# jedison-github/gentun

Measured on AMD Instinct MI355X. Metric: candidates/hour + best val-acc@genN, Genetic-CNN CIFAR-10 1/2/4/8 GPU, higher is better.
Workload: dtype fp32

## Files before the change

### csrc/hip/cnn_dense.hip

```cpp

#include <algorithm>
#include <cstdlib>

#include "common.h"

#define HEAD_MAXC_FWD 16
#define ADAM_B1 0.9f
#define ADAM_B2 0.999f
#define ADAM_EPS 1e-7f
#define CLIP_EPS 1e-7f
#define GT_DGRAD_BUF 2
#define GT_ADAM_UNROLL 1

__global__ void step_begin_kernel(StepState* s) {
  s->cur_step = s->step_ctr;
  s->step_ctr += 1;
  s->global_step += 1;
  const float t = s->t + 1.0f;
  s->t = t;
  s->lr_t = s->opt == 1 ? s->lr : s->lr * sqrtf(1.0f - powf(ADAM_B2, t)) / (1.0f - powf(ADAM_B1, t));
}

struct DenseFwdArgs {
  const void* x;
// ... 245 lines not shown
  const StepState* st;
  float* dH;
  float* gw2;
  float* gb2;
  float* gb1;
  float* eval_out;
  float* dz;
  const float* plog;
  int G, B, Up, C;
  int loss_ce;
  float drop_scale;
  int eval;
  int prec;
  const int* valid;
  const int* valid_norm;
  uint16_t* dHp;
};

#define HEAD_MAXB 64
#define HEAD_MAXC 16

__global__ void __launch_bounds__(64) head_fwd_kernel(HeadArgs a) {
  const int idx = blockIdx.x, lane = threadIdx.x;
  const int g = idx / a.B, b = idx % a.B;
  const int C = a.C, nt = a.Up / 16;
  const int step = a.st ? a.st->cur_step : 0;
  const long sid = a.gather[((long)step * a.G + g) * a.B + b];
  const int y = (int)a.labels[sid];
  float acc[HEAD_MAXC];
  const float* pl = a.plog + ((long)g * nt * a.B + b) * C;
#pragma unroll
  for (int c = 0; c < HEAD_MAXC; ++c) acc[c] = 0.f;
  for (int t = lane; t < nt; t += 64) {
    float v[HEAD_MAXC];
#pragma unroll
    for (int c = 0; c < HEAD_MAXC; ++c) v[c] = pl[(long)t * a.B * C + min(c, C - 1)];
#pragma unroll
    for (int c = 0; c < HEAD_MAXC; ++c) acc[c] += c < C ? v[c] : 0.f;
  }
#pragma unroll
  for (int c = 0; c < HEAD_MAXC; ++c) {
    if (c < C) {
#pragma unroll
      for (int o = 32; o > 0; o >>= 1) acc[c] += __shfl_xor(acc[c], o);
    }
  }
  if (lane != 0) return;
  float logit[HEAD_MAXC];
  for (int c = 0; c < C; ++c) logit[c] = acc[c] + a.b2[(long)g * C + c];
  float p[HEAD_MAXC];
  float mx = -INFINITY;
  for (int c = 0; c < C; ++c) mx = fmaxf(mx, logit[c]);
  float z = 0.f;
  for (int c = 0; c < C; ++c) { p[c] = expf(logit[c] - mx); z += p[c]; }
  int arg = 0;
  float loss = 0.f, binc = 0.f;
  for (int c = 0; c < C; ++c) {
    p[c] /= z;
    if (p[c] > p[arg]) arg = c;
    const float yc = (c == y) ? 1.f : 0.f;
    binc += (rintf(p[c]) == yc) ? 1.f : 0.f;
    if (!a.loss_ce) {
      const float pc = fminf(fmaxf(p[c], CLIP_EPS), 1.f - CLIP_EPS);
      loss += -(yc * logf(pc) + (1.f - yc) * logf(1.f - pc)) / C;
    }
  }
  if (a.loss_ce) loss = -logf(fmaxf(p[y], 1e-30f));
  if (a.eval) {
    float* e = a.eval_out + ((long)g * a.B + b) * 3;
    e[0] = loss; e[1] = binc; e[2] = (arg == y) ? 1.f : 0.f;
    return;
  }
  float* dz = a.dz + ((long)g * a.B + b) * C;
  const int nv = a.valid ? a.valid[(long)step * a.G + g] : a.B;
  const int nn = a.valid_norm ? a.valid_norm[(long)step * a.G + g] : nv;
  const float inv_b = (b < nv && nn > 0) ? 1.0f / nn : 0.f;
  if (a.loss_ce) {
    for (int c = 0; c < C; ++c) dz[c] = (p[c] - ((c == y) ? 1.f : 0.f)) * inv_b;
  } else {
    float dp[HEAD_MAXC], s = 0.f;
    for (int c = 0; c < C; ++c) {
      const float yc = (c == y) ? 1.f : 0.f;
      const bool inside = p[c] >= CLIP_EPS && p[c] <= 1.f - CLIP_EPS;
      const float pc = fminf(fmaxf(p[c], CLIP_EPS), 1.f - CLIP_EPS);
      dp[c] = inside ? (pc - yc) / (pc * (1.f - pc)) / C : 0.f;
      s += p[c] * dp[c];
    }
    for (int c = 0; c < C; ++c) dz[c] = p[c] * (dp[c] - s) * inv_b;
  }
}

__global__ void __launch_bounds__(256) head_bwd_kernel(HeadArgs a) {
  __shared__ float dzs[HEAD_MAXB * HEAD_MAXC];
  __shared__ float w2s[64 * HEAD_MAXC];
  __shared__ float hsl[HEAD_MAXB][65];
  __shared__ float colsum[4][64];
  const int g = blockIdx.y, u0 = blockIdx.x * 64, tid = threadIdx.x;
  const int B = a.B, Up = a.Up, C = a.C;
  const float* dz = a.dz + (long)g * B * C;
  for (int i = tid; i < B * C; i += 256) dzs[i] = dz[i];
  for (int i = tid; i < 64 * C; i += 256) {
    const int u = u0 + i / C;
    w2s[i] = (u < Up) ? a.w2[((long)g * Up + u0) * C + i] : 0.f;
  }
  for (int i = tid; i < B * 64; i += 256) {
    const int b = i >> 6, j = i & 63;
    const long hi = ((long)g * B + b) * Up + u0 + j;
    hsl[b][j] = (u0 + j < Up) ? (a.prec ? static_cast<const float*>(a.h)[hi] : bf2f(static_cast<const uint16_t*>(a.h)[hi]))
                              : 0.f;
  }
  __syncthreads();
  {
    const int j = tid & 63, q = tid >> 6;
    float sb = 0.f;
    for (int b = q; b < B; b += 4) {
      float s = 0.f;
      for (int c = 0; c < C; ++c) s += dzs[b * C + c] * w2s[j * C + c];
      const float d = hsl[b][j] > 0.f ? s * a.drop_scale : 0.f;
      if (u0 + j < Up) {
        const long o = ((long)g * B + b) * Up + u0 + j;
        a.dH[o] = d;
        if (a.dHp) {
          if (a.prec) {
            uint16_t hq[3];
            split3(d, hq);
            const long ps = (long)a.G * B * Up;
            a.dHp[o] = hq[0]; a.dHp[ps + o] = hq[1]; a.dHp[2 * ps + o] = hq[2];
          } else {
            a.dHp[o] = f2bf(d);
          }
        }
      }
      sb += d;
    }
    colsum[q][j] = sb;
  }
  for (int o = tid; o < 64 * C; o += 256) {
    const int j = o / C, c = o % C;
    if (u0 + j >= Up) continue;
    float s = 0.f;
    for (int b = 0; b < B; ++b) s += hsl[b][j] * dzs[b * C + c];
    a.gw2[((long)g * Up + u0) * C + o] = s;
  }
  __syncthreads();
  if (tid < 64 && u0 + tid < Up)
    a.gb1[(long)g * Up + u0 + tid] = colsum[0][tid] + colsum[1][tid] + colsum[2][tid] + colsum[3][tid];
  if (blockIdx.x == 0 && tid < C) {
    float s = 0.f;
    for (int b = 0; b < B; ++b) s += dzs[b * C + tid];
    a.gb2[(long)g * C + tid] = s;
  }
}

struct DenseDgradArgs {
  const float* dH;
  const void* wt;
  void* dx;
  int G, B, Fp, Up;
  int prec;
  long wps;
  const uint8_t* unpool_mask;
  void* unpool_x0;
  void* unpool_x1;
  const int* unpool_sel;
  int Hs, Ws, Cp;
  const float* w1;
  const uint16_t* dHp;
};

template <int PREC>
__device__ __forceinline__ void dense_dgrad_epilogue(const DenseDgradArgs& a, int g, int f_t, int b0,
                                                     const f32x4_t (&acc)[2], int lane) {
  typedef typename ActT<PREC>::T AT;
  const int kq = lane >> 4, l16 = lane & 15;
  const int fo = f_t + kq * 4;
  if (fo >= a.Fp) return;
#pragma unroll
  for (int h = 0; h < 2; ++h) {
    const int row = b0 + h * 16 + l16;
    if (row >= a.B) continue;
    float v[4] = {acc[h][0], acc[h][1], acc[h][2], acc[h][3]};
    if (a.unpool_mask) {
      const long n = (long)g * a.B + row;
      const int pix = fo / a.Cp, c0 = fo - pix * a.Cp, wo_n = a.Ws >> 1;
      const int ho = pix / wo_n, wo = pix - ho * wo_n;
      const uint32_t mk = *reinterpret_cast<const uint32_t*>(a.unpool_mask + n * a.Fp + fo);
      AT* src = static_cast<AT*>((a.unpool_sel && a.unpool_sel[g]) ? a.unpool_x1 : a.unpool_x0);
#pragma unroll
      for (int me = 0; me < 4; ++me) {
        float o[4];
#pragma unroll
        for (int j = 0; j < 4; ++j) {
          const uint32_t bb = (mk >> (8 * j)) & 0xffu;
          o[j] = ((int)(bb & 3u) == me && (bb & 4u)) ? v[j] : 0.f;
        }
        AT* d = src + ((n * a.Hs + 2 * ho + (me >> 1)) * a.Ws + 2 * wo + (me & 1)) * a.Cp + c0;
        if (PREC) *reinterpret_cast<float4*>(d) = make_float4(o[0], o[1], o[2], o[3]);
        else *reinterpret_cast<uint2*>(d) = pack4(o);
      }
      continue;
    }
    AT* dst = static_cast<AT*>(a.dx) + ((long)g * a.B + row) * a.Fp + fo;
    if (PREC) *reinterpret_cast<float4*>(dst) = make_float4(v[0], v[1], v[2], v[3]);
    else *reinterpret_cast<uint2*>(dst) = pack4(v);
  }
}

template <int PREC>
__global__ void __launch_bounds__(256) dense_dgrad_stream2_kernel(DenseDgradArgs a) {
  constexpr int NPL = PREC ? GT_NPL_F32 : 1;
  const int tid = threadIdx.x, wave = tid >> 6, lane = tid & 63, kq = lane >> 4, l16 = lane & 15;
  int bx, g;
  xcd_tile(bx, g);
  const int f_t = bx * 128 + wave * 32;
  const int b0 = blockIdx.y * 32;
  const float* wrow[2];
  bool fok[2];
#pragma unroll
  for (int m = 0; m < 2; ++m) {
    const int fa = f_t + 16 * m + l16;
    fok[m] = fa < a.Fp;
    wrow[m] = a.w1 + ((long)g * a.Fp + (fok[m] ? fa : 0)) * a.Up;
  }
  const long ps = (long)a.G * a.B * a.Up;
  const int br[2] = {b0 + l16, b0 + 16 + l16};
  const uint16_t* hp[2];
  bool bok[2];
#pragma unroll
  for (int h = 0; h < 2; ++h) {
    bok[h] = br[h] < a.B;
    hp[h] = a.dHp + ((long)g * a.B + (bok[h] ? br[h] : 0)) * a.Up;
  }
  const int nchunks = a.Up >> 3;
  const int nks = (nchunks + 3) >> 2;
  f32x4_t acc[2][2];
#pragma unroll
  for (int m = 0; m < 2; ++m) acc[m][0] = acc[m][1] = (f32x4_t){0.f, 0.f, 0.f, 0.f};
  constexpr int NBUF = GT_DGRAD_BUF;
  float rw[NBUF][2][8];
  uint4 rh[NBUF][2][NPL];
  const uint4* zero4 = reinterpret_cast<const uint4*>(gt_zero8);
  auto load = [&](int j, int buf) {
    const int c = 4 * j + kq;
    const bool cok = c < nchunks;
#pragma unroll
    for (int m = 0; m < 2; ++m) ld8_raw(wrow[m] + c * 8, cok && fok[m], rw[buf][m]);
#pragma unroll
    for (int h = 0; h < 2; ++h)
#pragma unroll
      for (int p = 0; p < NPL; ++p)
        rh[buf][h][p] = *((cok && bok[h]) ? reinterpret_cast<const uint4*>(hp[h] + p * ps + c * 8) : zero4);
  };
  auto step = [&](int buf) {
#pragma unroll
    for (int m = 0; m < 2; ++m) {
      uint4 af[NPL];
      planes8<PREC>(rw[buf][m], af);
      acc[m][0] = mfma_np<NPL>(af, rh[buf][0], acc[m][0]);
      acc[m][1] = mfma_np<NPL>(af, rh[buf][1], acc[m][1]);
    }
  };
#pragma unroll
  for (int t = 0; t < NBUF; ++t) {
    load(t, t);
    __builtin_amdgcn_sched_barrier(0);
  }
  const int nks2 = (nks + 1) & ~1;
  for (int j = 0; j < nks; j += NBUF) {
#pragma unroll
    for (int t = 0; t < NBUF; ++t) {
      if (j + t < nks2) step(t);
      __builtin_amdgcn_sched_barrier(0);
      load(j + NBUF + t, t);
      __builtin_amdgcn_sched_barrier(0);
    }
  }
#pragma unroll
  for (int m = 0; m < 2; ++m) dense_dgrad_epilogue<PREC>(a, g, f_t + 16 * m, b0, acc[m], lane);
}


__device__ __forceinline__ f32x4_t mfma4f(float a, float b, f32x4_t c) {
  return __builtin_amdgcn_mfma_f32_16x16x4f32(a, b, c, 0, 0, 0);
}

__global__ void __launch_bounds__(256) dense_dgrad_f32_kernel(DenseDgradArgs a) {
  const int tid = threadIdx.x, wave = tid >> 6, lane = tid & 63, kq = lane >> 4, l16 = lane & 15;
  int bx, g;
  xcd_tile(bx, g);
  const int f_t = bx * 128 + wave * 32;
  const int b0 = blockIdx.y * 32;
  const float* wrow[2];
#pragma unroll
  for (int m = 0; m < 2; ++m) wrow[m] = a.w1 + ((long)g * a.Fp + min(f_t + 16 * m + l16, a.Fp - 1)) * a.Up + 8 * kq;
  const float* hrow[2];
#pragma unroll
  for (int h = 0; h < 2; ++h) hrow[h] = a.dH + ((long)g * a.B + min(b0 + 16 * h + l16, a.B - 1)) * a.Up + 8 * kq;
  f32x4_t acc[2][2];
#pragma unroll
  for (int m = 0; m < 2; ++m) acc[m][0] = acc[m][1] = (f32x4_t){0.f, 0.f, 0.f, 0.f};
  constexpr int NB = 2;
  float4 wv[NB][2][2], hv[NB][2][2];
  const int nblk = a.Up >> 5;
  auto load = [&](int j, int buf) {
    const int jj = min(j, nblk - 1);
#pragma unroll
    for (int m = 0; m < 2; ++m) {
      wv[buf][m][0] = *reinterpret_cast<const float4*>(wrow[m] + 32 * jj);
      wv[buf][m][1] = *reinterpret_cast<const float4*>(wrow[m] + 32 * jj + 4);
    }
#pragma unroll
    for (int h = 0; h < 2; ++h) {
      hv[buf][h][0] = *reinterpret_cast<const float4*>(hrow[h] + 32 * jj);
      hv[buf][h][1] = *reinterpret_cast<const float4*>(hrow[h] + 32 * jj + 4);
    }
  };
  auto step = [&](int buf) {
#pragma unroll
    for (int q = 0; q < 8; ++q) {
      const float w0 = (&wv[buf][0][q >> 2].x)[q & 3], w1 = (&wv[buf][1][q >> 2].x)[q & 3];
      const float h0 = (&hv[buf][0][q >> 2].x)[q & 3], h1 = (&hv[buf][1][q >> 2].x)[q & 3];
      acc[0][0] = mfma4f(w0, h0, acc[0][0]);
      acc[0][1] = mfma4f(w0, h1, acc[0][1]);
      acc[1][0] = mfma4f(w1, h0, acc[1][0]);
      acc[1][1] = mfma4f(w1, h1, acc[1][1]);
    }
  };
#pragma unroll
  for (int i = 0; i < NB - 1; ++i) load(i, i);
  for (int j = 0; j < nblk; j += NB) {
#pragma unroll
    for (int q = 0; q < NB; ++q) {
      if (j + q >= nblk) break;
      load(j + q + NB - 1, (q + NB - 1) % NB);
      step(q);
    }
  }
#pragma unroll
  for (int m = 0; m < 2; ++m) dense_dgrad_epilogue<1>(a, g, f_t + 16 * m, b0, acc[m], lane);
}

struct DenseWgradAdamArgs {
  const void* x;
  const float* dH;
  float* p; float* m; float* v;
  void* wt;
  const StepState* st;
  int G, B, Fp, Up;
  int Cp, Cr, Ur;
  int prec;
  long wps;
  float* gbuf;
  int mode;
};

template <int PREC>
__global__ void __launch_bounds__(256) dense_wgrad_adam_kernel(DenseWgradAdamArgs a) {
  typedef typename ActT<PREC>::T AT;
  extern __shared__ __attribute__((aligned(16))) char smem[];
  float* xs = reinterpret_cast<float*>(smem);
  const int g = blockIdx.y, f0 = blockIdx.x * 16, tid = threadIdx.x;
  const AT* x = static_cast<const AT*>(a.x) + (long)g * a.B * a.Fp;
  for (int i = tid; i < a.B * 16; i += 256) {
    const int b = i >> 4, j = i & 15;
    float xv = 0.f;
    if (f0 + j < a.Fp) {
      if (PREC) xv = static_cast<const float*>(static_cast<const void*>(x))[(long)b * a.Fp + f0 + j];
      else xv = bf2f(static_cast<const uint16_t*>(static_cast<const void*>(x))[(long)b * a.Fp + f0 + j]);
    }
    xs[i] = xv;
  }
  __syncthreads();
  const float lr_t = a.st->lr_t;
  const float* dH = a.dH + (long)g * a.B * a.Up;
  const int nq = a.Ur > 0 ? (a.Ur + 3) >> 2 : a.Up >> 2;
  const int fr = tid >> 7;
  for (int q = tid & 127; q < nq; q += 128) {
    const int u0 = q * 4;
    float acc[8][4];
#pragma unroll
    for (int r = 0; r < 8; ++r) acc[r][0] = acc[r][1] = acc[r][2] = acc[r][3] = 0.f;
    if (a.mode == 2) {
#pragma unroll
      for (int r = 0; r < 8; ++r) {
        const int f = f0 + fr + 2 * r;
        if (f < a.Fp) {
          const float4 q4 = *reinterpret_cast<const float4*>(a.gbuf + ((long)g * a.Fp + f) * a.Up + u0);
          acc[r][0] = q4.x; acc[r][1] = q4.y; acc[r][2] = q4.z; acc[r][3] = q4.w;
        }
      }
    }
    for (int b = 0; a.mode != 2 && b < a.B; ++b) {
      const float4 d = *reinterpret_cast<const float4*>(dH + (long)b * a.Up + u0);
#pragma unroll
      for (int r = 0; r < 8; ++r) {
        const float xv = xs[b * 16 + fr + 2 * r];
        acc[r][0] += xv * d.x; acc[r][1] += xv * d.y; acc[r][2] += xv * d.z; acc[r][3] += xv * d.w;
      }
    }
    if (a.mode == 1) {
#pragma unroll
      for (int r = 0; r < 8; ++r) {
        const int f = f0 + fr + 2 * r;
        if (f < a.Fp)
          *reinterpret_cast<float4*>(a.gbuf + ((long)g * a.Fp + f) * a.Up + u0) =
              make_float4(acc[r][0], acc[r][1], acc[r][2], acc[r][3]);
      }
      continue;
    }
#pragma unroll
    for (int r = 0; r < 8; ++r) {
      const int f = f0 + fr + 2 * r;
      if (f >= a.Fp) continue;
      if (a.Cp > 0 && f % a.Cp >= a.Cr) continue;
      const long off = ((long)g * a.Fp + f) * a.Up + u0;
      float4 pp = *reinterpret_cast<float4*>(a.p + off);
      float4 mm = *reinterpret_cast<float4*>(a.m + off);
      float4 vv = *reinterpret_cast<float4*>(a.v + off);
      float* P = &pp.x; float* M = &mm.x; float* V = &vv.x;
#pragma unroll
      for (int i = 0; i < 4; ++i) P[i] = opt_update(a.st, P[i], acc[r][i], M[i], V[i], lr_t);
      *reinterpret_cast<float4*>(a.p + off) = pp;
      *reinterpret_cast<float4*>(a.m + off) = mm;
      *reinterpret_cast<float4*>(a.v + off) = vv;
    }
  }
}

struct AdamSeg {
  float* p; float* m; float* v;
  const float* g;
  uint16_t* bf;
  uint16_t* bfT;
  long n, gstride;
  int S, tG, tCo, tKH, tKW, tCi;
  int tiled;
  int npl;
  long pstride_bf, pstride_bfT;
};


#define ADAM_TK 64
#define ADAM_BLK 1024

struct AdamArgs {
  const AdamSeg* segs;
  const int2* blocks;
  const StepState* st;
};

__global__ void __launch_bounds__(256) adam_segments_kernel(AdamArgs a) {
  const int2 blk = a.blocks[blockIdx.x];
  const AdamSeg sg = a.segs[blk.x];
  const int npl = sg.npl > 1 ? GT_NPL_F32 : 1;
  if (sg.tiled) {
    __shared__ __attribute__((aligned(16))) uint16_t tile[GT_NPL_F32][ADAM_TK][128 + 8];
    const int CoF = sg.tCo, Ci = sg.tCi, KH = sg.tKH, KW = sg.tKW;
    const int Kd = KH * KW * Ci;
    const int nkt = (Kd + ADAM_TK - 1) / ADAM_TK;
    const int ncot = (CoF + 127) >> 7;
    const int gb = blk.y / nkt, k0 = (blk.y - gb * nkt) * ADAM_TK;
    const int gg = gb / ncot, c0 = (gb - gg * ncot) << 7;
    const int Co = min(128, CoF - c0);
    const long base = ((long)gg * CoF + c0) * Kd;
    const float lr_t = a.st->lr_t;
    constexpr int U = GT_ADAM_UNROLL;
    for (int idx0 = threadIdx.x; idx0 < Co * ADAM_TK; idx0 += 256 * U) {
      float gr[U], mv[U], vv[U], pv[U];
      long iv[U];
      bool ok[U];
#pragma unroll
      for (int u = 0; u < U; ++u) {
        const int idx = idx0 + 256 * u;
        const int co = idx / ADAM_TK, kk = idx % ADAM_TK, k = k0 + kk;
        ok[u] = idx < Co * ADAM_TK && k < Kd;
        iv[u] = base + (long)co * Kd + (ok[u] ? k : 0);
        gr[u] = 0.f; mv[u] = vv[u] = pv[u] = 0.f;
        if (ok[u]) {
          for (int s = 0; s < sg.S; ++s) gr[u] += sg.g[(long)s * sg.gstride + iv[u]];
          mv[u] = sg.m[iv[u]]; vv[u] = sg.v[iv[u]]; pv[u] = sg.p[iv[u]];
        }
      }
#pragma unroll
      for (int u = 0; u < U; ++u) {
        if (!ok[u]) continue;
        const int idx = idx0 + 256 * u;
        const int co = idx / ADAM_TK, kk = idx % ADAM_TK;
        const long i = iv[u];
        float m = mv[u], v = vv[u];
        const float p = opt_update(a.st, pv[u], gr[u], m, v, lr_t);
        sg.m[i] = m; sg.v[i] = v; sg.p[i] = p;
        uint16_t h[3];
        split3(p, h);
        for (int q = 0; q < npl; ++q) {
          if (sg.bf) sg.bf[q * sg.pstride_bf + i] = h[q];
          tile[q][kk][co] = h[q];
        }
      }
    }
    __syncthreads();
    const int nc8 = Co >> 3;
    for (int idx = threadIdx.x; idx < ADAM_TK * nc8; idx += 256) {
      const int kk = idx / nc8, c8 = idx - kk * nc8, k = k0 + kk;
      if (k >= Kd) continue;
      const int ci = k % Ci, r = k / Ci, kw = r % KW, kh = r / KW;
      const long o = ((((long)gg * Ci + ci) * KH + (KH - 1 - kh)) * KW + (KW - 1 - kw)) * CoF + c0 + c8 * 8;
      for (int q = 0; q < npl; ++q)
        *reinterpret_cast<uint4*>(sg.bfT + q * sg.pstride_bfT + o) = *reinterpret_cast<const uint4*>(&tile[q][kk][c8 * 8]);
    }
    return;
  }
  const float lr_t = a.st->lr_t;
  const int i0 = blk.y;
  auto one = [&](int i, float gr, float p, float& m, float& v) {
    p = opt_update(a.st, p, gr, m, v, lr_t);
    uint16_t h[3];
    split3(p, h);
    if (sg.bf)
      for (int q = 0; q < npl; ++q) sg.bf[q * sg.pstride_bf + i] = h[q];
    if (sg.bfT) {
      uint32_t r = (uint32_t)i;
      const uint32_t ci = r % (uint32_t)sg.tCi; r /= (uint32_t)sg.tCi;
      const uint32_t kw = r % (uint32_t)sg.tKW; r /= (uint32_t)sg.tKW;
      const uint32_t kh = r % (uint32_t)sg.tKH; r /= (uint32_t)sg.tKH;
      const uint32_t co = r % (uint32_t)sg.tCo;
      const uint32_t gg = r / (uint32_t)sg.tCo;
      const long o = ((((long)gg * sg.tCi + ci) * sg.tKH + (sg.tKH - 1 - kh)) * sg.tKW + (sg.tKW - 1 - kw)) * sg.tCo + co;
      for (int q = 0; q < npl; ++q) sg.bfT[q * sg.pstride_bfT + o] = h[q];
    }
    return p;
  };
  const bool vec = ((reinterpret_cast<uintptr_t>(sg.p) | reinterpret_cast<uintptr_t>(sg.m) |
                     reinterpret_cast<uintptr_t>(sg.v) | reinterpret_cast<uintptr_t>(sg.g)) & 15) == 0 &&
                   (sg.gstride & 3) == 0 && (long)i0 + ADAM_BLK <= sg.n;
  if (vec) {
    const int i = i0 + 4 * (int)threadIdx.x;
    float4 gr = make_float4(0.f, 0.f, 0.f, 0.f);
    for (int s = 0; s < sg.S; ++s) {
      const float4 t = *reinterpret_cast<const float4*>(sg.g + (long)s * sg.gstride + i);
      gr.x += t.x; gr.y += t.y; gr.z += t.z; gr.w += t.w;
    }
    float4 m = *reinterpret_cast<const float4*>(sg.m + i), v = *reinterpret_cast<const float4*>(sg.v + i);
    float4 p = *reinterpret_cast<const float4*>(sg.p + i);
    p.x = one(i, gr.x, p.x, m.x, v.x);
    p.y = one(i + 1, gr.y, p.y, m.y, v.y);
    p.z = one(i + 2, gr.z, p.z, m.z, v.z);
    p.w = one(i + 3, gr.w, p.w, m.w, v.w);
    *reinterpret_cast<float4*>(sg.m + i) = m;
    *reinterpret_cast<float4*>(sg.v + i) = v;
    *reinterpret_cast<float4*>(sg.p + i) = p;
    return;
  }
  for (int e = 0; e < ADAM_BLK / 256; ++e) {
    const int i = i0 + e * 256 + (int)threadIdx.x;
    if (i >= sg.n) return;
    float gr = 0.f;
    for (int s = 0; s < sg.S; ++s) gr += sg.g[(long)s * sg.gstride + i];
    float m = sg.m[i], v = sg.v[i];
    const float p = one(i, gr, sg.p[i], m, v);
    sg.m[i] = m; sg.v[i] = v; sg.p[i] = p;
  }
}

extern "C" {

int gt_step_begin(StepState* s, hipStream_t stream) {
  hipLaunchKernelGGL(step_begin_kernel, dim3(1), dim3(1), 0, stream, s);
  return (int)hipGetLastError();
}

int gt_dense_fwd_splits(int Fp) {
  const int nks = (Fp + 31) / 32;
  return std::max(1, std::min(16, nks / 12));
}

int gt_dense_fwd(const DenseFwdArgs* a, hipStream_t stream) {
  if (a->Fp % 8 || a->Up % 64 || a->C > HEAD_MAXC_FWD || (a->prec != 0 && a->prec != 1)) return -1;
  if (!a->w1 || a->ks < 1 || (a->ks > 1 && !a->part)) return -3;
  dim3 grid(a->Up / 64 * a->ks, (a->B + 31) / 32, a->G);
  if (a->prec) hipLaunchKernelGGL(dense_fwd_sk_kernel<1>, grid, dim3(256), 0, stream, *a);
  else hipLaunchKernelGGL(dense_fwd_sk_kernel<0>, grid, dim3(256), 0, stream, *a);
  if (a->ks > 1) {
    dim3 rgrid(a->Up / 64, (a->B + 31) / 32, a->G);
    if (a->prec) hipLaunchKernelGGL(dense_fwd_skred_kernel<1>, rgrid, dim3(256), 0, stream, *a);
    else hipLaunchKernelGGL(dense_fwd_skred_kernel<0>, rgrid, dim3(256), 0, stream, *a);
  }
  return (int)hipGetLastError();
}

int gt_head(const HeadArgs* a, hipStream_t stream) {
  if ((!a->eval && a->B > HEAD_MAXB) || a->C > HEAD_MAXC) return -1;
  if (a->Up % 16) return -2;
  hipLaunchKernelGGL(head_fwd_kernel, dim3(a->G * a->B), dim3(64), 0, stream, *a);
  if (!a->eval) hipLaunchKernelGGL(head_bwd_kernel, dim3((a->Up + 63) / 64, a->G), dim3(256), 0, stream, *a);
  return (int)hipGetLastError();
}

int gt_dense_dgrad(const DenseDgradArgs* a, hipStream_t stream) {
  if (a->Fp % 64 && a->Fp % 8) return -1;
  if (a->unpool_mask && (a->Cp % 8 || a->Hs % 2 || a->Ws % 2 || (long)(a->Hs / 2) * (a->Ws / 2) * a->Cp != a->Fp))
    return -1;
  if (a->Up % 8) return -1;
  if (a->prec != 0 && a->prec != 1) return -1;
  if (!a->w1) return -3;
  dim3 grid((a->Fp + 127) / 128, (a->B + 31) / 32, a->G);
  if (a->prec == 1) {
    if (a->Up % 32) return -1;
    hipLaunchKernelGGL(dense_dgrad_f32_kernel, grid, dim3(256), 0, stream, *a);
  } else {
    if (!a->dHp) return -3;
    hipLaunchKernelGGL(dense_dgrad_stream2_kernel<0>, grid, dim3(256), 0, stream, *a);
  }
  return (int)hipGetLastError();
}

int gt_dense_wgrad_adam(const DenseWgradAdamArgs* a, hipStream_t stream) {
  if (a->Up % 4 || (a->prec != 0 && a->prec != 1)) return -1;
  const size_t lds = sizeof(float) * (size_t)a->B * 16;
  if (lds > 160 * 1024) return -2;
  dim3 grid((a->Fp + 15) / 16, a->G);
  if (a->prec) {
    if (lds > 65536) (void)hipFuncSetAttribute(reinterpret_cast<const void*>(dense_wgrad_adam_kernel<1>),
                                         hipFuncAttributeMaxDynamicSharedMemorySize, (int)lds);
    hipLaunchKernelGGL(dense_wgrad_adam_kernel<1>, grid, dim3(256), lds, stream, *a);
  } else {
    hipLaunchKernelGGL(dense_wgrad_adam_kernel<0>, grid, dim3(256), lds, stream, *a);
  }
  return (int)hipGetLastError();
}

int gt_adam_segments(const AdamArgs* a, int nblocks, hipStream_t stream) {
  hipLaunchKernelGGL(adam_segments_kernel, dim3(nblocks), dim3(256), 0, stream, *a);
  return (int)hipGetLastError();
}

size_t gt_sizeof_adam_seg() { return sizeof(AdamSeg); }
int gt_adam_block_elems() { return ADAM_BLK; }
size_t gt_sizeof_dense_fwd_args() { return sizeof(DenseFwdArgs); }
size_t gt_sizeof_head_args() { return sizeof(HeadArgs); }
size_t gt_sizeof_dense_dgrad_args() { return sizeof(DenseDgradArgs); }
size_t gt_sizeof_dense_wgrad_args() { return sizeof(DenseWgradAdamArgs); }

}
```

### gentun_amd/ops/cnn_kernels.py

```python

import ctypes as C
import os

from . import _lib

P = C.c_void_p
I = C.c_int


MAXSLOT = 8

PREC = {"bf16": 0, "fp32": 1}
NPL = {"bf16": 1, "fp32": 3}


class GroupRec(C.Structure):
    _fields_ = [("g", I), ("in_mask", I), ("out_mask", I), ("pad", I)]


class ConvArgs(C.Structure):
    _fields_ = [("inp", P * MAXSLOT), ("mask", P), ("gather", P), ("st", P), ("out", P * MAXSLOT),
                ("out_mask", P * MAXSLOT), ("w", P), ("bias", P), ("gtab", P),
                ("n_in", I), ("n_out", I), ("acc_flags", I), ("relu", I),
                ("G", I), ("B", I), ("H", I), ("W", I), ("Cinp", I), ("Coutp", I), ("KH", I), ("KW", I),
# ... 90 lines not shown


class HeadArgs(C.Structure):
    _fields_ = [("h", P), ("w2", P), ("b2", P), ("labels", P), ("gather", P), ("st", P), ("dH", P),
                ("gw2", P), ("gb2", P), ("gb1", P), ("eval_out", P), ("dz", P), ("plog", P),
                ("G", I), ("B", I), ("Up", I), ("C", I), ("loss_ce", I), ("drop_scale", C.c_float), ("eval", I),
                ("prec", I), ("valid", P), ("valid_norm", P), ("dHp", P)]


class DenseDgradArgs(C.Structure):
    _fields_ = [("dH", P), ("wt", P), ("dx", P), ("G", I), ("B", I), ("Fp", I), ("Up", I), ("prec", I),
                ("wps", C.c_long), ("unpool_mask", P), ("unpool_x0", P), ("unpool_x1", P), ("unpool_sel", P),
                ("Hs", I), ("Ws", I), ("Cp", I), ("w1", P), ("dHp", P)]


class DenseWgradAdamArgs(C.Structure):
    _fields_ = [("x", P), ("dH", P), ("p", P), ("m", P), ("v", P), ("wt", P), ("st", P),
                ("G", I), ("B", I), ("Fp", I), ("Up", I), ("Cp", I), ("Cr", I), ("Ur", I), ("prec", I),
                ("wps", C.c_long), ("gbuf", P), ("mode", I)]


class AdamSeg(C.Structure):
    _fields_ = [("p", P), ("m", P), ("v", P), ("g", P), ("bf", P), ("bfT", P), ("n", C.c_long),
                ("gstride", C.c_long), ("S", I), ("tG", I), ("tCo", I), ("tKH", I), ("tKW", I), ("tCi", I),
                ("tiled", I), ("npl", I), ("pstride_bf", C.c_long), ("pstride_bfT", C.c_long)]

ADAM_TK = 64


ADAM_BLK = 1024


def adam_blocks(n):
    return range(0, n, ADAM_BLK)


def adam_tiles(tG, tCo, tKH, tKW, tCi):
    if tCo % 8:
        return 0
    kd = tKH * tKW * tCi
    return tG * (-(-tCo // 128)) * (-(-kd // ADAM_TK))


class BnArgs(C.Structure):
    _fields_ = [("z", P), ("y", P), ("gamma", P), ("beta", P), ("stat", P), ("run", P), ("part", P),
                ("ggamma", P), ("gbeta", P), ("gtab", P), ("valid", P), ("st", P),
                ("ngroups", I), ("G", I), ("B", I), ("HW", I), ("Cp", I), ("nchunk", I), ("chunk_px", I),
                ("momentum", C.c_float), ("eps", C.c_float), ("train", I), ("prec", I),
                ("pool_y", P), ("pool_mask", P), ("W", I), ("Hr", I), ("Wr", I)]


BN_CHUNK_PX = 512
BN_CHUNK_VALUES = 16384


def bn_chunk_px(H, W, Cp):
    c = BN_CHUNK_PX
    pooled = BN_CHUNK_PX % (2 * W) == 0
    while c * Cp > BN_CHUNK_VALUES and (c // 2 >= 2 * W and (c // 2) % (2 * W) == 0 if pooled else c > 64):
        c //= 2
    return c


class AdamArgs(C.Structure):
    _fields_ = [("segs", P), ("blocks", P), ("st", P)]


class ProgOp(C.Structure):
    _fields_ = [("kind", C.c_int32), ("stream", C.c_int32), ("event", C.c_int32), ("pad", C.c_int32),
                ("v", C.c_int64 * 14)]


PROG_OPS = {"record": 0, "wait": 1, "gt_step_begin": 2, "gt_conv_fwd": 3, "gt_conv_wgrad": 4,
            "gt_wgrad_reduce": 5, "gt_bn_fwd": 6, "gt_bn_bwd": 7, "gt_dense_fwd": 8, "gt_head": 9,
            "gt_dense_dgrad": 10, "gt_dense_wgrad_adam": 11, "gt_adam_segments": 12, "gt_pool_fwd": 13,
            "gt_pool_fwd_mask": 14, "gt_pool_bwd_mask": 15, "gt_wino_wtrans": 16,
            "gt_conv_wfrag": 17}


class InitSeg(C.Structure):
    _fields_ = [("p", P), ("seeds", P), ("d", I * 4), ("r", I * 4), ("G", I), ("tag", I), ("limit", C.c_float),
                ("pad", I)]


class InitArgs(C.Structure):
    _fields_ = [("segs", P), ("blocks", P)]


_TYPED = {}


def lib():
    L = _lib.hip()
    if not _TYPED.get(id(L)):
        for name, argt in (("gt_conv_fwd", C.POINTER(ConvArgs)), ("gt_conv_wgrad", C.POINTER(WgradArgs)),
                           ("gt_dense_fwd", C.POINTER(DenseFwdArgs)), ("gt_head", C.POINTER(HeadArgs)),
                           ("gt_dense_dgrad", C.POINTER(DenseDgradArgs)),
                           ("gt_dense_wgrad_adam", C.POINTER(DenseWgradAdamArgs))):
            fn = getattr(L, name)
            fn.argtypes = [argt, P]
            fn.restype = I
        for name in ("gt_bn_fwd", "gt_bn_bwd"):
            fn = getattr(L, name)
            fn.argtypes = [C.POINTER(BnArgs), P]
            fn.restype = I
        L.gt_adam_segments.argtypes = [C.POINTER(AdamArgs), I, P]
        L.gt_adam_segments.restype = I
        L.gt_step_begin.argtypes = [P, P]
        L.gt_step_begin.restype = I
        L.gt_pool_fwd.argtypes = [P, P, P, P, I, I, I, I, I, I, P]
        L.gt_pool_fwd.restype = I
        L.gt_pool_bwd.argtypes = [P, P, P, P, P, P, I, I, I, I, I, I, I, P]
        L.gt_pool_bwd.restype = I
        L.gt_pool_fwd_mask.argtypes = [P, P, P, P, I, I, I, I, I, P, I, P]
        L.gt_pool_fwd_mask.restype = I
        L.gt_pool_bwd_mask.argtypes = [P, P, P, P, P, I, I, I, I, I, I, I, P]
        L.gt_pool_bwd_mask.restype = I
        L.gt_wgrad_set_nb.argtypes = [I]
        L.gt_wgrad_set_nb.restype = I
        L.gt_wgrad_fast_band.argtypes = [I, I, I, I, I, I, I]
        L.gt_wgrad_fast_splits.argtypes = [I, I, I, I, I, I, I]
        L.gt_wgrad_fast_splits.restype = I
        L.gt_wgrad_fast_band.restype = I
        L.gt_conv_fast_probe.argtypes = [C.POINTER(ConvArgs)]
        L.gt_conv_fast_probe.restype = I
        L.gt_conv_fast_probe_any.argtypes = [C.POINTER(ConvArgs)]
        L.gt_conv_fast_probe_any.restype = I
        L.gt_wgrad_reduce.argtypes = [C.POINTER(WgradArgs), P]
        L.gt_wgrad_reduce.restype = I
        L.gt_conv_frag_order.argtypes = [I, I, I, I, I, C.POINTER(C.c_int), I]
        L.gt_conv_frag_order.restype = I
        L.gt_conv_wfrag.argtypes = [P, I, P]
        L.gt_conv_wfrag.restype = I
        L.gt_sizeof_frag_seg.restype = C.c_size_t
        assert L.gt_sizeof_frag_seg() == C.sizeof(FragSeg), "FragSeg ABI mismatch"
        L.gt_conv_wino_supported.argtypes = [I, I, I, I]
        L.gt_conv_wino_supported.restype = I
        L.gt_wino_wtrans.argtypes = [P, I, P]
        L.gt_wino_wtrans.restype = I
        L.gt_sizeof_wino_wseg.restype = C.c_size_t
        assert L.gt_sizeof_wino_wseg() == C.sizeof(WinoWSeg), "WinoWSeg ABI mismatch"
        L.gt_conv_set_fast.argtypes = [I]
        L.gt_conv_set_fast.restype = I
        L.gt_conv_set_nwv.argtypes = [I]
        L.gt_conv_set_s2in_ct1.restype = I
        L.gt_dense_fwd_splits.argtypes = [I]
        L.gt_dense_fwd_splits.restype = I
        L.gt_conv_set_smallq.argtypes = [I]
        L.gt_conv_set_smallq.restype = I
        L.gt_conv_set_s2in_ct1.argtypes = [I]
        L.gt_conv_set_nwv.restype = I
        L.gt_conv_set_imgs.argtypes = [I]
        L.gt_conv_set_imgs.restype = I
        L.gt_glorot_init.argtypes = [C.POINTER(InitArgs), I, P]
        L.gt_glorot_init.restype = I
        L.gt_glorot_ref.argtypes = [C.c_uint64, C.c_uint64, I, C.c_float]
        L.gt_glorot_ref.restype = C.c_float
        L.gt_prog_create.argtypes = [C.POINTER(ProgOp), I, I, I]
        L.gt_prog_create.restype = P
        L.gt_prog_run.argtypes = [P, P, I, C.POINTER(I)]
        L.gt_prog_run.restype = I
        L.gt_prog_destroy.argtypes = [P]
        L.gt_prog_destroy.restype = None
        L.gt_sizeof_prog_op.restype = C.c_size_t
        assert L.gt_sizeof_prog_op() == C.sizeof(ProgOp), "ProgOp ABI mismatch"
        for name in ("gt_sizeof_conv_args", "gt_sizeof_wgrad_args", "gt_sizeof_adam_seg", "gt_sizeof_init_seg",
                     "gt_sizeof_dense_fwd_args", "gt_sizeof_head_args", "gt_sizeof_dense_dgrad_args",
                     "gt_sizeof_dense_wgrad_args", "gt_sizeof_bn_args"):
            getattr(L, name).restype = C.c_size_t
        assert L.gt_sizeof_conv_args() == C.sizeof(ConvArgs), "ConvArgs ABI mismatch"
        assert L.gt_sizeof_init_seg() == C.sizeof(InitSeg), "InitSeg ABI mismatch"
        assert L.gt_sizeof_wgrad_args() == C.sizeof(WgradArgs), "WgradArgs ABI mismatch"
        assert L.gt_sizeof_adam_seg() == C.sizeof(AdamSeg), "AdamSeg ABI mismatch"
        assert L.gt_adam_block_elems() == ADAM_BLK, "Adam block size mismatch"
        assert L.gt_sizeof_bn_args() == C.sizeof(BnArgs), "BnArgs ABI mismatch"
        for nm, st in (("dense_fwd_args", DenseFwdArgs), ("head_args", HeadArgs),
                       ("dense_dgrad_args", DenseDgradArgs), ("dense_wgrad_args", DenseWgradAdamArgs)):
            assert getattr(L, "gt_sizeof_" + nm)() == C.sizeof(st), nm + " ABI mismatch"
        _TYPED[id(L)] = True
    return L


def check(rc, what):
    if rc != 0:
        raise RuntimeError("HIP kernel launch {} failed with code {}".format(what, rc))


class StepProgram(object):

    def __init__(self, plan):
        L = lib()
        self.L = L
        keys, nev = [None], 0
        ops = (ProgOp * len(plan))()
        for o, op in zip(ops, plan):
            st = op[3] if op[0] == "k" else op[1]
            if not any(st is k for k in keys):
                keys.append(st)
            o.stream = next(i for i, k in enumerate(keys) if k is st)
            if op[0] in ("rec", "wait"):
                o.kind = PROG_OPS["record" if op[0] == "rec" else "wait"]
                o.event = int(op[2])
                nev = max(nev, o.event + 1)
                continue
            o.kind = PROG_OPS[op[1]]
            vals = []
            for a in op[2]:
                if isinstance(a, C.Structure):
                    vals.append(C.addressof(a))
                elif a is None:
                    vals.append(0)
                elif isinstance(a, C.c_void_p):
                    vals.append(a.value or 0)
                else:
                    vals.append(int(a))
            if len(vals) > len(o.v):
                raise ValueError("step program: too many operands for " + op[1])
            for i, x in enumerate(vals):
                o.v[i] = x
        self._ops = ops
        self._structs = [a for op in plan if op[0] == "k" for a in op[2] if isinstance(a, C.Structure)]
        self.keys = keys
        self.h = L.gt_prog_create(ops, len(plan), nev, len(keys))
        if not self.h:
            raise RuntimeError("gt_prog_create rejected the step program")
        self._streams = (C.c_void_p * len(keys))()

    def run(self, main_stream, nsteps):
        self._streams[0] = main_stream
        for i, k in enumerate(self.keys[1:], 1):
            self._streams[i] = k.cuda_stream
        bad = I(-1)
        rc = self.L.gt_prog_run(self.h, self._streams, int(nsteps), C.byref(bad))
        if rc != 0:
            raise RuntimeError("HIP step program op {} failed with code {}".format(bad.value, rc))

    def __del__(self):
        h, self.h = getattr(self, "h", None), None
        if h:
            try:
                self.L.gt_prog_destroy(h)
            except Exception:
                pass


def ptr(t):
    return C.c_void_p(t.data_ptr()) if t is not None else C.c_void_p(0)


CONV_TILE_PIXELS = 128


def conv_tile_rows(H, W, tile_pixels=None):
    tp = tile_pixels or CONV_TILE_PIXELS
    if W > tp:
        raise ValueError("image width > {} not supported by conv_fwd tiles".format(tp))
    return max(1, min(H, tp // W))


def wino_segment(master, planes, dgrad):
    Q, cop, kh, kw, cip = master.shape
    assert (kh, kw) == (3, 3) and master.dtype.is_floating_point and master.is_contiguous()
    R, Kc = (wino_dims(cop, cip) if dgrad else wino_dims(cip, cop))
    assert tuple(planes.shape) == (3, Q, 16, R, Kc) and planes.is_contiguous(), (planes.shape, (3, Q, 16, R, Kc))
    sg = WinoWSeg()
    sg.w, sg.u, sg.ups = master.data_ptr(), planes.data_ptr(), planes[0].numel()
    sg.Q, sg.Cop, sg.Cip, sg.R, sg.K, sg.dgrad = Q, cop, cip, R, Kc, 1 if dgrad else 0
    return sg


class WinoTransform(object):

    def __init__(self, segs, device):
        import numpy as np
        import torch
        self.nseg = len(segs)
        blocks = []
        for i, sg in enumerate(segs):
            n = sg.Q * sg.R * sg.K
            blocks.extend((i, o) for o in range(0, n, 256))
        arr = (WinoWSeg * max(1, len(segs)))(*segs)
        self.segs_t = torch.frombuffer(bytearray(bytes(memoryview(arr).cast("B"))), dtype=torch.uint8).to(device)
        self.blocks_t = torch.tensor(np.asarray(blocks, np.int32).reshape(-1, 2), device=device)
        self.args = WinoWArgs()
        self.args.segs, self.args.blocks = self.segs_t.data_ptr(), self.blocks_t.data_ptr()
        self.nblocks = len(blocks)

    def run(self, stream):
        if self.nblocks:
            check(lib().gt_wino_wtrans(C.addressof(self.args), self.nblocks, stream), "wino_wtrans")


def wino_unpack(planes):
    npl, Q, nxi, R, Kc = planes.shape
    f = planes.reshape(npl, Q, nxi, R // 16, Kc // 32, 4, 16, 8)
    return f.permute(0, 1, 2, 3, 6, 4, 5, 7).reshape(npl, Q, nxi, R, Kc)


def wino_weights(master, dgrad=False, stream=None):
    import torch
    Q, cop, _, _, cip = master.shape
    R, Kc = wino_dims(cop, cip) if dgrad else wino_dims(cip, cop)
    planes = torch.zeros((3, Q, 16, R, Kc), dtype=torch.bfloat16, device=master.device)
    tr = WinoTransform([wino_segment(master.contiguous(), planes, dgrad)], master.device)
    tr.run(torch.cuda.current_stream(master.device).cuda_stream if stream is None else stream)
    tr.keep = planes
# ... 98 lines not shown
```

Before: 1066.

## Fuse head forward/backward into one kernel and add LDS-staged dense wgrad+Adam

Adds a fused head training kernel that reduces the split-K partial logits, computes softmax and the loss gradient, and produces dH, gw2, gb1 and gb2 in one launch instead of separate forward and backward kernels. Also adds a persistent fp32 dense weight-gradient plus Adam kernel. It stages dH slices in LDS, double-buffers x tiles, and prefetches the next tile's p/m/v while computing the current one. Both paths are on by default behind runtime toggles, and the old kernels remain as fallbacks. The risks are a large per-thread register array in the logit reduction, redundant softmax recomputation in every block, and a grid capped at 256 workgroups.

```diff
diff --git a/csrc/hip/cnn_dense.hip b/csrc/hip/cnn_dense.hip
--- a/csrc/hip/cnn_dense.hip
+++ b/csrc/hip/cnn_dense.hip
@@ -421,6 +421,139 @@
   }
 }
 
+__global__ void __launch_bounds__(256) head_train_kernel(HeadArgs a) {
+  __shared__ float dzs[HEAD_MAXB * HEAD_MAXC];
+  __shared__ float w2s[64 * HEAD_MAXC];
+  __shared__ float hsl[HEAD_MAXB][65];
+  __shared__ float colsum[4][64];
+  __shared__ float lgs[HEAD_MAXB][HEAD_MAXC + 1];
+  const int g = blockIdx.y, u0 = blockIdx.x * 64, tid = threadIdx.x;
+  const int B = a.B, Up = a.Up, C = a.C;
+  const int step = a.st ? a.st->cur_step : 0;
+  int y = 0, nv = B, nn = B;
+  if (tid < B) {
+    const long sid = a.gather[((long)step * a.G + g) * B + tid];
+    y = (int)a.labels[sid];
+    nv = a.valid ? a.valid[(long)step * a.G + g] : B;
+    nn = a.valid_norm ? a.valid_norm[(long)step * a.G + g] : nv;
+  }
+  for (int i = tid; i < 64 * C; i += 256) {
+    const int u = u0 + i / C;
+    w2s[i] = (u < Up) ? a.w2[((long)g * Up + u0) * C + i] : 0.f;
+  }
+  for (int i = tid; i < B * 64; i += 256) {
+    const int b = i >> 6, j = i & 63;
+    const long hi = ((long)g * B + b) * Up + u0 + j;
+    hsl[b][j] = (u0 + j < Up) ? (a.prec ? static_cast<const float*>(a.h)[hi] : bf2f(static_cast<const uint16_t*>(a.h)[hi]))
+                              : 0.f;
+  }
+  {
+    const int nt = Up / 16, bc = B * C;
+    for (int i = tid; i < bc; i += 256) {
+      const float* pl = a.plog + (long)g * nt * bc + i;
+      float l[64];
+#pragma unroll
+      for (int t = 0; t < 64; ++t) l[t] = pl[(long)min(t, nt - 1) * bc];
+#pragma unroll
+      for (int t = 0; t < 64; ++t) l[t] = t < nt ? 0.f + l[t] : 0.f;
+#pragma unroll
+      for (int o = 32; o > 0; o >>= 1) {
+#pragma unroll
+        for (int t = 0; t < o; ++t) l[t] = l[t] + l[t + o];
+      }
+      lgs[i / C][i % C] = l[0];
+    }
+  }
+  __syncthreads();
+  if (tid < B) {
+    const int b = tid;
+    float p[HEAD_MAXC];
+    float mx = -INFINITY;
+#pragma unroll
+    for (int c = 0; c < HEAD_MAXC; ++c) {
+      p[c] = c < C ? lgs[b][c] + a.b2[(long)g * C + min(c, C - 1)] : 0.f;
+      if (c < C) mx = fmaxf(mx, p[c]);
+    }
+    float z = 0.f;
+#pragma unroll
+    for (int c = 0; c < HEAD_MAXC; ++c)
+      if (c < C) { p[c] = expf(p[c] - mx); z += p[c]; }
+#pragma unroll
+    for (int c = 0; c < HEAD_MAXC; ++c)
+      if (c < C) p[c] /= z;
+    const float inv_b = (b < nv && nn > 0) ? 1.0f / nn : 0.f;
+    float dzr[HEAD_MAXC];
+    if (a.loss_ce) {
+#pragma unroll
+      for (int c = 0; c < HEAD_MAXC; ++c) dzr[c] = (p[c] - ((c == y) ? 1.f : 0.f)) * inv_b;
+    } else {
+      float dp[HEAD_MAXC], s = 0.f;
+#pragma unroll
+      for (int c = 0; c < HEAD_MAXC; ++c) {
+        dp[c] = 0.f;
+        if (c < C) {
+          const float yc = (c == y) ? 1.f : 0.f;
+          const bool inside = p[c] >= CLIP_EPS && p[c] <= 1.f - CLIP_EPS;
+          const float pc = fminf(fmaxf(p[c], CLIP_EPS), 1.f - CLIP_EPS);
+          dp[c] = inside ? (pc - yc) / (pc * (1.f - pc)) / C : 0.f;
+          s += p[c] * dp[c];
+        }
+      }
+#pragma unroll
+      for (int c = 0; c < HEAD_MAXC; ++c) dzr[c] = p[c] * (dp[c] - s) * inv_b;
+    }
+    float* dz = a.dz + ((long)g * B + b) * C;
+#pragma unroll
+    for (int c = 0; c < HEAD_MAXC; ++c) {
+      if (c < C) {
+        dzs[b * C + c] = dzr[c];
+        if (blockIdx.x == 0) dz[c] = dzr[c];
+      }
+    }
+  }
+  __syncthreads();
+  {
+    const int j = tid & 63, q = tid >> 6;
+    float sb = 0.f;
+    for (int b = q; b < B; b += 4) {
+      float s = 0.f;
+      for (int c = 0; c < C; ++c) s += dzs[b * C + c] * w2s[j * C + c];
+      const float d = hsl[b][j] > 0.f ? s * a.drop_scale : 0.f;
+      if (u0 + j < Up) {
+        const long o = ((long)g * B + b) * Up + u0 + j;
+        a.dH[o] = d;
+        if (a.dHp) {
+          if (a.prec) {
+            uint16_t hq[3];
+            split3(d, hq);
+            const long ps = (long)a.G * B * Up;
+            a.dHp[o] = hq[0]; a.dHp[ps + o] = hq[1]; a.dHp[2 * ps + o] = hq[2];
+          } else {
+            a.dHp[o] = f2bf(d);
+          }
+        }
+      }
+      sb += d;
+    }
+    colsum[q][j] = sb;
+  }
+  for (int o = tid; o < 64 * C; o += 256) {
+    const int j = o / C, c = o % C;
+    if (u0 + j >= Up) continue;
+    float s = 0.f;
+    for (int b = 0; b < B; ++b) s += hsl[b][j] * dzs[b * C + c];
+    a.gw2[((long)g * Up + u0) * C + o] = s;
+  }
+  __syncthreads();
+  if (tid < 64 && u0 + tid < Up)
+    a.gb1[(long)g * Up + u0 + tid] = colsum[0][tid] + colsum[1][tid] + colsum[2][tid] + colsum[3][tid];
+  if (blockIdx.x == 0 && tid < C) {
+    float s = 0.f;
+    for (int b = 0; b < B; ++b) s += dzs[b * C + tid];
+    a.gb2[(long)g * C + tid] = s;
+  }
+}
+
 struct DenseDgradArgs {
   const float* dH;
   const void* wt;
@@ -693,6 +826,138 @@
       *reinterpret_cast<float4*>(a.m + off) = mm;
       *reinterpret_cast<float4*>(a.v + off) = vv;
     }
+  }
+}
+
+#define DWL_SW 256
+#define DWL_MAXB 32
+#define DWL_MAXWG 256
+#define DWL_BC 2
+
+__global__ void __launch_bounds__(256) dense_wgrad_adam_lds_kernel(DenseWgradAdamArgs a) {
+  __shared__ __attribute__((aligned(16))) float dHs[DWL_MAXB * DWL_SW];
+  __shared__ float xs[2][DWL_MAXB * 16];
+  const int tid = threadIdx.x, ql = tid & 63;
+  const int w = __builtin_amdgcn_readfirstlane(tid >> 6);
+  const int B = a.B, Fp = a.Fp, Up = a.Up;
+  const int ntile = (Fp + 15) >> 4, nsl = (Up + DWL_SW - 1) / DWL_SW;
+  const long nitem = (long)a.G * nsl * ntile;
+  const int beg = (int)(nitem * blockIdx.x / gridDim.x), end = (int)(nitem * (blockIdx.x + 1) / gridDim.x);
+  if (beg >= end) return;
+  const int nq = a.Ur > 0 ? (a.Ur + 3) >> 2 : Up >> 2;
+  const float lr_t = a.st->lr_t;
+
+  auto decode = [&](int it, int& gs, int& f0) { gs = it / ntile; f0 = (it - gs * ntile) << 4; };
+  auto unit0 = [&](int gs) { const int u = (gs % nsl) * DWL_SW + ql * 4; return (u >> 2) < nq && u < Up ? u : -1; };
+  auto row_ok = [&](int f) { return f < Fp && !(a.Cp > 0 && f % a.Cp >= a.Cr); };
+  auto load_x = [&](int gs, int f0, float* xr) {
+    const float* x = static_cast<const float*>(a.x) + (long)(gs / nsl) * B * Fp;
+#pragma unroll
+    for (int e = 0; e < 2; ++e) {
+      const int i = tid + 256 * e, b = i >> 4, j = i & 15;
+      xr[e] = (b < B && f0 + j < Fp) ? x[(long)b * Fp + f0 + j] : 0.f;
+    }
+  };
+  auto load_pmv = [&](int gs, int f0, float4* P, float4* M, float4* V) {
+    const int u0 = unit0(gs);
+#pragma unroll
+    for (int r = 0; r < 4; ++r) {
+      const int f = f0 + w + 4 * r;
+      if (u0 >= 0 && row_ok(f)) {
+        const long off = ((long)(gs / nsl) * Fp + f) * Up + u0;
+        P[r] = *reinterpret_cast<const float4*>(a.p + off);
+        M[r] = *reinterpret_cast<const float4*>(a.m + off);
+        V[r] = *reinterpret_cast<const float4*>(a.v + off);
+      }
+    }
+  };
+
+  float xr[2];
+  float4 P[4], M[4], V[4];
+  int gs, f0, staged = -1, buf = 0;
+  decode(beg, gs, f0);
+  load_x(gs, f0, xr);
+  load_pmv(gs, f0, P, M, V);
+  for (int it = beg; it < end; ++it) {
+    if (gs != staged) {
+      __syncthreads();
+      const float* dH = a.dH + (long)(gs / nsl) * B * Up;
+      const int us = (gs % nsl) * DWL_SW;
+      const int u = us + ql * 4;
+      float4 dv[DWL_MAXB / 4];
+#pragma unroll
+      for (int e = 0; e < DWL_MAXB / 4; ++e) {
+        const int b = w + 4 * e;
+        dv[e] = (b < B && u < Up) ? *reinterpret_cast<const float4*>(dH + (long)b * Up + u) : make_float4(0.f, 0.f, 0.f, 0.f);
+      }
+#pragma unroll
+      for (int e = 0; e < DWL_MAXB / 4; ++e) *reinterpret_cast<float4*>(dHs + (w + 4 * e) * DWL_SW + ql * 4) = dv[e];
+      staged = gs;
+    }
+#pragma unroll
+    for (int e = 0; e < 2; ++e) {
+      const int i = tid + 256 * e;
+      if (i < B * 16) xs[buf][i] = xr[e];
+    }
+    __syncthreads();
+    const int gs_c = gs, f0_c = f0;
+    float4 Pn[4], Mn[4], Vn[4];
+    if (it + 1 < end) {
+      decode(it + 1, gs, f0);
+      load_x(gs, f0, xr);
+      load_pmv(gs, f0, Pn, Mn, Vn);
+    }
+    const int u0 = unit0(gs_c);
+    if (u0 >= 0) {
+      float acc[4][4];
+#pragma unroll
+      for (int r = 0; r < 4; ++r) acc[r][0] = acc[r][1] = acc[r][2] = acc[r][3] = 0.f;
+      const float* dq = dHs + ql * 4;
+      const float* xb = xs[buf] + w;
+      int b = 0;
+      for (; b + DWL_BC <= B; b += DWL_BC) {
+        float4 d[DWL_BC];
+        float xv[DWL_BC][4];
+#pragma unroll
+        for (int j = 0; j < DWL_BC; ++j) {
+          d[j] = *reinterpret_cast<const float4*>(dq + (b + j) * DWL_SW);
+#pragma unroll
+          for (int r = 0; r < 4; ++r) xv[j][r] = xb[(b + j) * 16 + 4 * r];
+        }
+#pragma unroll
+        for (int j = 0; j < DWL_BC; ++j) {
+#pragma unroll
+          for (int r = 0; r < 4; ++r) {
+            acc[r][0] += xv[j][r] * d[j].x; acc[r][1] += xv[j][r] * d[j].y;
+            acc[r][2] += xv[j][r] * d[j].z; acc[r][3] += xv[j][r] * d[j].w;
+          }
+        }
+      }
+      for (; b < B; ++b) {
+        const float4 d = *reinterpret_cast<const float4*>(dq + b * DWL_SW);
+#pragma unroll
+        for (int r = 0; r < 4; ++r) {
+          const float xv = xb[b * 16 + 4 * r];
+          acc[r][0] += xv * d.x; acc[r][1] += xv * d.y; acc[r][2] += xv * d.z; acc[r][3] += xv * d.w;
+        }
+      }
+#pragma unroll
+      for (int r = 0; r < 4; ++r) {
+        const int f = f0_c + w + 4 * r;
+        if (!row_ok(f)) continue;
+        const long off = ((long)(gs_c / nsl) * Fp + f) * Up + u0;
+        float4 pp = P[r], mm = M[r], vv = V[r];
+        float* Pp = &pp.x; float* Mp = &mm.x; float* Vp = &vv.x;
+#pragma unroll
+        for (int i = 0; i < 4; ++i) Pp[i] = opt_update(a.st, Pp[i], acc[r][i], Mp[i], Vp[i], lr_t);
+        *reinterpret_cast<float4*>(a.p + off) = pp;
+        *reinterpret_cast<float4*>(a.m + off) = mm;
+        *reinterpret_cast<float4*>(a.v + off) = vv;
+      }
+    }
+#pragma unroll
+    for (int r = 0; r < 4; ++r) { P[r] = Pn[r]; M[r] = Mn[r]; V[r] = Vn[r]; }
+    buf ^= 1;
   }
 }
 
@@ -831,6 +1096,9 @@
   }
 }
 
+static int g_head_fused = 1;
+static int g_dense_w1_lds = 1;
+
 extern "C" {
 
 int gt_step_begin(StepState* s, hipStream_t stream) {
@@ -860,9 +1128,25 @@
 int gt_head(const HeadArgs* a, hipStream_t stream) {
   if ((!a->eval && a->B > HEAD_MAXB) || a->C > HEAD_MAXC) return -1;
   if (a->Up % 16) return -2;
+  if (!a->eval && g_head_fused && a->Up <= 1024) {
+    hipLaunchKernelGGL(head_train_kernel, dim3((a->Up + 63) / 64, a->G), dim3(256), 0, stream, *a);
+    return (int)hipGetLastError();
+  }
   hipLaunchKernelGGL(head_fwd_kernel, dim3(a->G * a->B), dim3(64), 0, stream, *a);
   if (!a->eval) hipLaunchKernelGGL(head_bwd_kernel, dim3((a->Up + 63) / 64, a->G), dim3(256), 0, stream, *a);
   return (int)hipGetLastError();
+}
+
+int gt_head_set_fused(int on) {
+  const int old = g_head_fused;
+  g_head_fused = on ? 1 : 0;
+  return old;
+}
+
+int gt_dense_wgrad_set_lds(int on) {
+  const int old = g_dense_w1_lds;
+  g_dense_w1_lds = on ? 1 : 0;
+  return old;
 }
 
 int gt_dense_dgrad(const DenseDgradArgs* a, hipStream_t stream) {
@@ -885,6 +1169,13 @@
 
 int gt_dense_wgrad_adam(const DenseWgradAdamArgs* a, hipStream_t stream) {
   if (a->Up % 4 || (a->prec != 0 && a->prec != 1)) return -1;
+  if (g_dense_w1_lds && a->prec == 1 && a->mode == 0 && a->B <= DWL_MAXB) {
+    const long nitem = (long)a->G * ((a->Up + DWL_SW - 1) / DWL_SW) * ((a->Fp + 15) / 16);
+    if (nitem < 1 || nitem > 0x7fffffffL) return -1;
+    hipLaunchKernelGGL(dense_wgrad_adam_lds_kernel, dim3((unsigned)std::min<long>(DWL_MAXWG, nitem)), dim3(256), 0,
+                       stream, *a);
+    return (int)hipGetLastError();
+  }
   const size_t lds = sizeof(float) * (size_t)a->B * 16;
   if (lds > 160 * 1024) return -2;
   dim3 grid((a->Fp + 15) / 16, a->G);
diff --git a/gentun_amd/ops/cnn_kernels.py b/gentun_amd/ops/cnn_kernels.py
--- a/gentun_amd/ops/cnn_kernels.py
+++ b/gentun_amd/ops/cnn_kernels.py
@@ -266,6 +266,10 @@
         L.gt_conv_set_nwv.restype = I
         L.gt_conv_set_imgs.argtypes = [I]
         L.gt_conv_set_imgs.restype = I
+        L.gt_head_set_fused.argtypes = [I]
+        L.gt_head_set_fused.restype = I
+        L.gt_dense_wgrad_set_lds.argtypes = [I]
+        L.gt_dense_wgrad_set_lds.restype = I
         L.gt_glorot_init.argtypes = [C.POINTER(InitArgs), I, P]
         L.gt_glorot_init.restype = I
         L.gt_glorot_ref.argtypes = [C.c_uint64, C.c_uint64, I, C.c_float]
```

New measurement: 1069, median of 6. About the same (+0.3%).
